# bigomics/plaid

Measured on NVIDIA B200. Metric: plaid() cells x genesets scored/sec, higher is better.
Workload: dtype f64

## Files before the change

### plaid_b200/csrc/api.cu

```cuda
#include <math.h>
#include <stdio.h>
#include <string.h>
#include <stdlib.h>
#include <time.h>
#if defined(__x86_64__)
#include <immintrin.h>
#endif

#include <algorithm>
#include <condition_variable>
#include <functional>
#include <mutex>
#include <new>
#include <thread>

#include "common.cuh"

using namespace plaidgpu;

namespace {

struct DevBuf {
  void* p = nullptr;
  size_t cap = 0;
// ... 667 lines not shown
  CK(c->b_rowb.reserve((size_t)c->P * sizeof(double)));
  const double* dmean = nullptr;
  if (mean_host) {
    CK(cudaMemcpyAsync(c->b_rowb.p, mean_host, (size_t)c->P * sizeof(double), cudaMemcpyHostToDevice, c->stream));
    dmean = c->b_rowb.as<double>();
  }
  CK(launch_row_moments(c->xx, c->P, c->N, dmean, c->b_rowa.as<double>(), c->stream));
  c->launches += 1;
  CK(cudaMemcpyAsync(out_host, c->b_rowa.p, (size_t)c->P * sizeof(double), cudaMemcpyDeviceToHost, c->stream));
  CK(cudaStreamSynchronize(c->stream));
  return PLAIDGPU_OK;
}

bool is_rank_scorer(int s) {
  return s == PLAIDGPU_SING || s == PLAIDGPU_SSGSEA || s == PLAIDGPU_UCELL || s == PLAIDGPU_AUCELL;
}

bool needs_norm(const plaidgpu_opts& o) {
  return (o.scorer == PLAIDGPU_PLAID && o.normalize) || o.scorer == PLAIDGPU_SSGSEA || o.scorer == PLAIDGPU_UCELL ||
         o.scorer == PLAIDGPU_AUCELL || o.scorer == PLAIDGPU_GSVA;
}

double host_value_of(unsigned long long k) {
  const unsigned long long b = (k & 0x8000000000000000ull) ? (k & 0x7fffffffffffffffull) : ~k;
  double d;
  memcpy(&d, &b, sizeof(d));
  return d;
}

int run_colstats(plaidgpu_ctx* c, int which) {
  CK(c->b_med_all.reserve(std::max<int64_t>(c->N, 1) * sizeof(double)));
  CK(c->b_med_nz.reserve(std::max<int64_t>(c->N, 1) * sizeof(double)));
  CK(c->b_colmin.reserve(std::max<int64_t>(c->N, 1) * sizeof(double)));
  CK(c->b_fail.reserve(sizeof(int)));
  CK(c->b_list.reserve(std::max<int64_t>(c->N, 1) * sizeof(int64_t)));
  CK(launch_colstats(c->raw, c->S, c->S, c->N, c->b_med_all.as<double>(), c->b_med_nz.as<double>(),
                     c->b_colmin.as<double>(), c->b_fail.as<int>(), c->b_list.as<int64_t>(), which, c->stream));
  c->launches += 1;
  if (which != COLSTATS_NZ) c->have_all = true;
  if (which != COLSTATS_ALL) c->have_nz = true;
  return PLAIDGPU_OK;
}

void ship_join(plaidgpu_ctx* c) {
  if (!c->shipper.joinable()) return;
  {
    std::lock_guard<std::mutex> lk(c->ship_m);
    c->ship_done = true;
  }
  c->ship_cv.notify_all();
  c->shipper.join();
}
void ship_body(plaidgpu_ctx* c) {
  cudaSetDevice(c->device);
  size_t next = 0;
  for (;;) {
    std::pair<int64_t, int64_t> job;
    {
      std::unique_lock<std::mutex> lk(c->ship_m);
      c->ship_cv.wait(lk, [&] { return next < c->ship_q.size() || c->ship_done; });
      if (next >= c->ship_q.size()) return;
      job = c->ship_q[next];
    }
    cudaStreamWaitEvent(c->copy_stream, c->ev_ship[next], 0);
    cudaMemcpyAsync(c->early_out + job.first * (int64_t)c->S, c->raw + job.first * (int64_t)c->S,
                    (size_t)job.second * c->S * sizeof(double), cudaMemcpyDeviceToHost, c->copy_stream);
    cudaEventRecord(c->ev_early, c->copy_stream);
// ... 1755 lines not shown
  const double* dx = x;
  if (location == PLAIDGPU_HOST) {
    const size_t total = (size_t)S * (size_t)N;
    CK(c->b_raw.reserve(total * sizeof(double)));
    CK(cudaMemcpyAsync(c->b_raw.p, x, total * sizeof(double), cudaMemcpyHostToDevice, c->stream));
    dx = c->b_raw.as<double>();
  }
  return topk_device(c, dx, S, N, k, decreasing != 0, idx, val);
} catch (const std::bad_alloc&) {
  return PLAIDGPU_ERR_NOMEM;
} catch (...) {
  return PLAIDGPU_ERR_ARG;
}

int plaidgpu_normalize_medians(plaidgpu_ctx* c, const double* x, int32_t S, int64_t N, int ignore_zero,
                               int location, double* out) try {
  if (!c) return PLAIDGPU_ERR_ARG;
  if (S <= 0 || N < 0 || (N > 0 && (!x || !out))) return fail(c, PLAIDGPU_ERR_ARG, "bad argument");
  trace("begin");
  CK(cudaSetDevice(c->device));
  c->in_call = false;
  c->computed = false;
  const int64_t total = (int64_t)S * N;
  const double* dx = x;
  if (location == PLAIDGPU_HOST) {
    CK(c->b_raw.reserve((size_t)std::max<int64_t>(total, 1) * sizeof(double)));
    if (total) CK(cudaMemcpyAsync(c->b_raw.p, x, (size_t)total * sizeof(double), cudaMemcpyHostToDevice, c->stream));
    dx = c->b_raw.as<double>();
  }
  CK(c->b_med_all.reserve(std::max<int64_t>(N, 1) * sizeof(double)));
  CK(c->b_med_nz.reserve(std::max<int64_t>(N, 1) * sizeof(double)));
  CK(c->b_colmin.reserve(std::max<int64_t>(N, 1) * sizeof(double)));
  CK(cudaEventRecord(c->ev[2], c->stream));
  CK(c->b_fail.reserve(sizeof(int)));
  CK(c->b_list.reserve(std::max<int64_t>(N, 1) * sizeof(int64_t)));
  const int which = ignore_zero < 0 ? COLSTATS_BOTH : (ignore_zero ? COLSTATS_NZ : COLSTATS_ALL);
  CK(launch_colstats(dx, S, S, N, c->b_med_all.as<double>(), c->b_med_nz.as<double>(), c->b_colmin.as<double>(),
                     c->b_fail.as<int>(), c->b_list.as<int64_t>(), which, c->stream));
  c->launches += 1;
  CK(cudaEventRecord(c->ev[3], c->stream));
  c->h_med_all.resize((size_t)N);
  c->h_med_nz.resize((size_t)N);
  c->h_colmin.resize((size_t)N);
  if (N) {
    CK(cudaMemcpyAsync(c->h_med_all.data(), c->b_med_all.p, (size_t)N * sizeof(double), cudaMemcpyDeviceToHost, c->stream));
    CK(cudaMemcpyAsync(c->h_med_nz.data(), c->b_med_nz.p, (size_t)N * sizeof(double), cudaMemcpyDeviceToHost, c->stream));
    CK(cudaMemcpyAsync(c->h_colmin.data(), c->b_colmin.p, (size_t)N * sizeof(double), cudaMemcpyDeviceToHost, c->stream));
  }
  CK(cudaStreamSynchronize(c->stream));
  float ms = 0.f;
  cudaEventElapsedTime(&ms, c->ev[2], c->ev[3]);
  c->ms[1] = ms;
  double mn = INFINITY;
  for (int64_t j = 0; j < N; ++j) mn = fmin(mn, c->h_colmin[j]);
  plaidgpu_scalars s{};
  plaidgpu_combine_medians(ignore_zero, mn, c->h_med_all.data(), c->h_med_nz.data(), N, &s);
  const double* med = s.ignore_zero ? c->b_med_nz.as<double>() : c->b_med_all.as<double>();
  CK(cudaEventRecord(c->ev[4], c->stream));
  if (location == PLAIDGPU_DEVICE) {
    CK(launch_fixup(dx, out, S, S, 0, N, med, s.med_mean, 1.0, nullptr, c->stream));
    c->launches += 1;
    CK(cudaEventRecord(c->ev[5], c->stream));
  } else {
    CK(launch_fixup(dx, c->b_raw.as<double>(), S, S, 0, N, med, s.med_mean, 1.0, nullptr, c->stream));
    c->launches += 1;
    CK(cudaEventRecord(c->ev[5], c->stream));
    if (total) CK(cudaMemcpyAsync(out, c->b_raw.p, (size_t)total * sizeof(double), cudaMemcpyDeviceToHost, c->stream));
// ... 13 lines not shown
```

### plaid_b200/csrc/stats_kernels.cu

```cuda
#include "common.cuh"

#include <math.h>
#include <stdio.h>
#include <stdlib.h>

namespace plaidgpu {

namespace {

constexpr int NT = 256;
constexpr int NBIN = 2048;
constexpr int NTGT = 4;
constexpr int CAND = 256;
constexpr int NDIG = 6;
constexpr unsigned long long ZERO_KEY = 0x8000000000000000ull;

__device__ __forceinline__ int digit_shift(int d) { return d < 5 ? 53 - 11 * d : 0; }
__device__ __forceinline__ int digit_bits(int d) { return d < 5 ? 11 : 9; }


struct BinHit { int bin; unsigned before, count; };
__device__ BinHit find_bin(const unsigned* __restrict__ hist, int nb, unsigned k, unsigned* __restrict__ part,
                           BinHit* __restrict__ slot) {
  const int tid = threadIdx.x, lane = tid & 31;
  const int per = nb / NT;
  unsigned sum = 0;
  for (int i = 0; i < per; ++i) sum += hist[tid * per + i];
  part[tid] = sum;
  __syncthreads();
  if (tid < 32) {
    unsigned loc = 0;
#pragma unroll
    for (int i = 0; i < NT / 32; ++i) loc += part[lane * (NT / 32) + i];
    unsigned incl = loc;
#pragma unroll
    for (int o = 1; o < 32; o <<= 1) {
      const unsigned v = __shfl_up_sync(FULL, incl, o);
// ... 18 lines not shown

struct StatsSmem {
  unsigned hist[NTGT][NBIN];
  unsigned long long cand[NTGT][CAND];
  unsigned long long prefix[NTGT];
  unsigned long long result[NTGT];
  unsigned k[NTGT];
  unsigned cnt[NTGT];
  unsigned ncand[NTGT];
  int active[NTGT];
  int depth[NTGT];
  unsigned red_u[NT / 32][3];
  unsigned long long red_k[NT / 32];
  unsigned nnan, nzero, nneg;
  unsigned long long minkey;
  unsigned part[NT];
  BinHit hit;
};

__device__ void pick_bin(StatsSmem& s, int g, int d) {
  const BinHit h = find_bin(s.hist[g], 1 << digit_bits(d), s.k[g], s.part, &s.hit);
  __syncthreads();
  if (threadIdx.x == 0) {
    s.prefix[g] |= (unsigned long long)h.bin << digit_shift(d);
    s.k[g] -= h.before;
    s.cnt[g] = h.count;
    s.depth[g] = d + 1;
  }
  __syncthreads();
}

__global__ void __launch_bounds__(NT) k_colstats(const double* __restrict__ x, int64_t ld, int32_t S,
                                                 int64_t N, const int64_t* __restrict__ cols,
                                                 double* __restrict__ med_all,
                                                 double* __restrict__ med_nz,
                                                 double* __restrict__ colmin) {
  extern __shared__ unsigned char smem_raw[];
  StatsSmem& s = *reinterpret_cast<StatsSmem*>(smem_raw);
  const int tid = threadIdx.x, lane = tid & 31, wid = tid >> 5;

  for (int64_t it = blockIdx.x; it < N; it += gridDim.x) {
    const int64_t j = cols ? cols[it] : it;
    const double* __restrict__ c = x + j * ld;

    for (int i = tid; i < NBIN; i += NT) s.hist[0][i] = 0;
    __syncthreads();
    unsigned nnan = 0, nzero = 0;
    unsigned long long mink = ~0ull;
    int runbin = -1;
    unsigned runcnt = 0;
    for (int l = tid; l < S; l += NT) {
      const double v = c[l];
      if (v != v) {
        ++nnan;
        continue;
      }
      const unsigned long long key = key_of(v);
      nzero += (key == ZERO_KEY);
      mink = key < mink ? key : mink;
      const int bin = (int)(key >> 53);
      if (bin != runbin) {
        if (runcnt) atomicAdd(&s.hist[0][runbin], runcnt);
        runbin = bin;
        runcnt = 0;
      }
      ++runcnt;
    }
    if (runcnt) atomicAdd(&s.hist[0][runbin], runcnt);
    __syncthreads();
    unsigned nneg = 0;
    for (int i = tid; i < NBIN / 2; i += NT) nneg += s.hist[0][i];
#pragma unroll
// ... 767 lines not shown
        }
#pragma unroll
        for (int o = 16; o > 0; o >>= 1) {
          le += __shfl_xor_sync(FULL, le, o);
          const unsigned long long t = __shfl_xor_sync(FULL, nx, o);
          nx = t < nx ? t : nx;
        }
        if (lane == 0) {
          atomicAdd(&s.cle, le);
          atomicMin(&s.nxt, nx);
        }
        __syncthreads();
        B = (qb < s.cle) ? A : s.nxt;
      }
    }
    if (tid == 0) {
      if (!good) {
        const int slot = atomicAdd(fail_count, 1);
        fail_list[slot] = j;
      } else {
        double m = NZ ? 0.0 : nan("");
        if (count > 0) {
          const double a = value_of(A), b = value_of(B);
          m = (count & 1u) ? a : (a + b) / 2.0;
        }
        med[j] = m;
        colmin[j] = s.minkey != ~0ull ? value_of(s.minkey) : INFINITY;
      }
    }
    __syncthreads();
  }
}

__global__ void __launch_bounds__(256) k_fixup(const double* __restrict__ x, double* __restrict__ out,
                                               int64_t ld, int32_t S, int64_t j0, int64_t j1,
                                               const double* __restrict__ med, double c, double alpha,
                                               const double* __restrict__ beta) {
  for (int64_t j = j0 + blockIdx.x; j < j1; j += gridDim.x) {
    const double shift = (med ? -med[j] : 0.0) + c;
    const double* __restrict__ xi = x + j * ld;
    double* __restrict__ oi = out + j * ld;
    const bool vec = ((((uintptr_t)xi) | ((uintptr_t)oi)) & 15) == 0;
    if (vec) {
      const int S2 = S >> 1;
      const double2* __restrict__ x2 = reinterpret_cast<const double2*>(xi);
      double2* __restrict__ o2 = reinterpret_cast<double2*>(oi);
      for (int l = threadIdx.x; l < S2; l += blockDim.x) {
        double2 v = __ldcs(x2 + l);
        v.x = __dmul_rn(alpha, __dadd_rn(v.x, shift));
        v.y = __dmul_rn(alpha, __dadd_rn(v.y, shift));
        if (beta) {
          v.x = __dadd_rn(v.x, beta[2 * l]);
          v.y = __dadd_rn(v.y, beta[2 * l + 1]);
        }
        __stcs(o2 + l, v);
      }
      if ((S & 1) && threadIdx.x == 0) {
        double v = __dmul_rn(alpha, __dadd_rn(xi[S - 1], shift));
        if (beta) v = __dadd_rn(v, beta[S - 1]);
        oi[S - 1] = v;
      }
    } else {
      for (int l = threadIdx.x; l < S; l += blockDim.x) {
        double v = __dmul_rn(alpha, __dadd_rn(xi[l], shift));
        if (beta) v = __dadd_rn(v, beta[l]);
        oi[l] = v;
// ... 106 lines not shown
  out[0] = res[0] == ~0ull ? INFINITY : value_of(res[0]);
  out[1] = res[1] == 0ull ? -INFINITY : value_of(res[1]);
}

}

bool colstats_small(int32_t S) { return S < 4 * SAMP; }

cudaError_t launch_colstats(const double* x, int64_t ld, int32_t S, int64_t N, double* med_all,
                            double* med_nz, double* colmin, int* d_fail, int64_t* d_list, int which, cudaStream_t st) {
  if (N <= 0) return cudaSuccess;
  {
    cudaError_t e = cudaFuncSetAttribute(k_colstats, cudaFuncAttributeMaxDynamicSharedMemorySize,
                                         (int)sizeof(StatsSmem));
    if (e != cudaSuccess) return e;
    const void* fast[3] = {(const void*)k_colstats_fast<true, true>, (const void*)k_colstats_fast<true, false>,
                           (const void*)k_colstats_fast<false, true>};
    for (int i = 0; i < 3; ++i) {
      e = cudaFuncSetAttribute(fast[i], cudaFuncAttributeMaxDynamicSharedMemorySize,
                               (int)(i == 0 ? sizeof(Stats2Smem) : STATS2_SMEM_ONE));
      if (e != cudaSuccess) return e;
    }
    e = cudaFuncSetAttribute(k_colstats_one<false>, cudaFuncAttributeMaxDynamicSharedMemorySize, (int)sizeof(Stats3Smem));
    if (e != cudaSuccess) return e;
    e = cudaFuncSetAttribute(k_colstats_one<true>, cudaFuncAttributeMaxDynamicSharedMemorySize, (int)sizeof(Stats3Smem));
    if (e != cudaSuccess) return e;
  }
  int dev = 0, sms = 148;
  cudaGetDevice(&dev);
  cudaDeviceGetAttribute(&sms, cudaDevAttrMultiProcessorCount, dev);
  if (S < 4 * SAMP) {
    int64_t grid = (int64_t)sms * 4;
    if (grid > N) grid = N;
    k_colstats<<<(unsigned)grid, NT, sizeof(StatsSmem), st>>>(x, ld, S, N, nullptr, med_all, med_nz, colmin);
    return cudaGetLastError();
  }
  cudaError_t e = launch_fill_u32(d_fail, 0u, 1, st);
  if (e != cudaSuccess) return e;
  int per_sm = 1;
  static const bool old_one = getenv("PLAIDGPU_COLSTATS_OLD") != nullptr;
  if (which != COLSTATS_BOTH && !old_one) {
    const size_t sm3 = sizeof(Stats3Smem);
    if (which == COLSTATS_ALL) cudaOccupancyMaxActiveBlocksPerMultiprocessor(&per_sm, k_colstats_one<false>, NT, sm3);
    else cudaOccupancyMaxActiveBlocksPerMultiprocessor(&per_sm, k_colstats_one<true>, NT, sm3);
    if (per_sm < 1) per_sm = 1;
    int64_t grid = (int64_t)sms * per_sm;
    if (grid > N) grid = N;
    if (which == COLSTATS_ALL)
      k_colstats_one<false><<<(unsigned)grid, NT, sm3, st>>>(x, ld, S, N, med_all, colmin, d_fail, d_list);
    else
      k_colstats_one<true><<<(unsigned)grid, NT, sm3, st>>>(x, ld, S, N, med_nz, colmin, d_fail, d_list);
    e = cudaGetLastError();
    if (e != cudaSuccess) return e;
  } else {
  const size_t smem = which == COLSTATS_BOTH ? sizeof(Stats2Smem) : STATS2_SMEM_ONE;
  if (which == COLSTATS_ALL)
    cudaOccupancyMaxActiveBlocksPerMultiprocessor(&per_sm, k_colstats_fast<true, false>, NT, smem);
  else if (which == COLSTATS_NZ)
    cudaOccupancyMaxActiveBlocksPerMultiprocessor(&per_sm, k_colstats_fast<false, true>, NT, smem);
  else
    cudaOccupancyMaxActiveBlocksPerMultiprocessor(&per_sm, k_colstats_fast<true, true>, NT, smem);
  if (per_sm < 1) per_sm = 1;
  int64_t grid = (int64_t)sms * per_sm;
  if (grid > N) grid = N;
  if (which == COLSTATS_ALL)
    k_colstats_fast<true, false><<<(unsigned)grid, NT, smem, st>>>(x, ld, S, N, med_all, med_nz, colmin, d_fail, d_list);
  else if (which == COLSTATS_NZ)
    k_colstats_fast<false, true><<<(unsigned)grid, NT, smem, st>>>(x, ld, S, N, med_all, med_nz, colmin, d_fail, d_list);
  else
    k_colstats_fast<true, true><<<(unsigned)grid, NT, smem, st>>>(x, ld, S, N, med_all, med_nz, colmin, d_fail, d_list);
  e = cudaGetLastError();
  if (e != cudaSuccess) return e;
  }
  int nfail = 0;
  e = cudaMemcpyAsync(&nfail, d_fail, sizeof(int), cudaMemcpyDeviceToHost, st);
  if (e != cudaSuccess) return e;
  e = cudaStreamSynchronize(st);
  if (e != cudaSuccess) return e;
  if (getenv("PLAIDGPU_TRACE_COLSTATS"))
    fprintf(stderr, "[plaidgpu] colstats: %d of %lld columns redone by the three-pass kernel\n", nfail, (long long)N);
  if (nfail > 0) {
    int64_t g2 = (int64_t)sms * 4;
    if (g2 > nfail) g2 = nfail;
    k_colstats<<<(unsigned)g2, NT, sizeof(StatsSmem), st>>>(x, ld, S, nfail, d_list, med_all, med_nz, colmin);
    e = cudaGetLastError();
    if (e != cudaSuccess) return e;
  }
  return cudaSuccess;
}

cudaError_t launch_fixup(const double* x, double* out, int64_t ld, int32_t S, int64_t j0, int64_t j1,
                         const double* med, double c, double alpha, const double* beta,
                         cudaStream_t st) {
  if (j1 <= j0) return cudaSuccess;
  int dev = 0, sms = 148;
  cudaGetDevice(&dev);
  cudaDeviceGetAttribute(&sms, cudaDevAttrMultiProcessorCount, dev);
  if (ld == S && (S & 1) == 0 && S >= FIX_CHUNK && ((((uintptr_t)(x + j0 * ld)) | ((uintptr_t)(out + j0 * ld))) & 15) == 0) {
    const int64_t chunks = ((j1 - j0) * (int64_t)S + FIX_CHUNK - 1) / FIX_CHUNK;
    int64_t grid = (int64_t)sms * 8;
    if (grid > chunks) grid = chunks;
    k_fixup_flat<<<(unsigned)grid, 256, 0, st>>>(x, out, S, j0, j1, med, c, alpha, beta);
    return cudaGetLastError();
  }
  int64_t grid = (int64_t)sms * 8;
  if (grid > j1 - j0) grid = j1 - j0;
  k_fixup<<<(unsigned)grid, 256, 0, st>>>(x, out, ld, S, j0, j1, med, c, alpha, beta);
  return cudaGetLastError();
}

cudaError_t launch_group_stats(const double* x, int64_t ld, int32_t S, int K, const int32_t* cols, const int32_t* seg,
                               int nchunk, double* partial, double* out, cudaStream_t st, bool fix, const double* med,
                               double c, double alpha, const double* beta) {
  if (S <= 0 || K <= 0) return cudaSuccess;
  dim3 g((unsigned)((int64_t)nchunk * K), (unsigned)((S + 255) / 256));
  if (fix) k_group_partial<true><<<g, 256, 0, st>>>(x, ld, S, cols, seg, partial, med, c, alpha, beta);
  else k_group_partial<false><<<g, 256, 0, st>>>(x, ld, S, cols, seg, partial, nullptr, 0.0, 1.0, nullptr);
  cudaError_t e = cudaGetLastError();
  if (e != cudaSuccess) return e;
  const int64_t width = (int64_t)K * 2 * S;
  k_group_combine<<<(unsigned)((width + 255) / 256), 256, 0, st>>>(partial, width, nchunk, out);
// ... 25 lines not shown
```

### plaid_b200/csrc/tail_kernels.cu

```cuda
#include "common.cuh"

namespace plaidgpu {

namespace {

constexpr int TAIL_WARPS = 32;

__global__ void __launch_bounds__(1024) k_tile_scan(uint32_t* __restrict__ cnt, int32_t Pt, uint32_t* __restrict__ rowptr,
                                                    uint32_t* __restrict__ total) {
  __shared__ uint32_t wsum[32];
  const int t = blockIdx.x, tid = threadIdx.x, lane = tid & 31, w = tid >> 5;
  uint32_t* __restrict__ c = cnt + (size_t)t * Pt;
  uint32_t* __restrict__ rp = rowptr + (size_t)t * (Pt + 1);
  const int per = (Pt + 1023) / 1024;
  const int lo = min(Pt, tid * per), hi = min(Pt, lo + per);
  uint32_t s = 0;
  for (int i = lo; i < hi; ++i) s += c[i];
  uint32_t incl = s;
#pragma unroll
  for (int o = 1; o < 32; o <<= 1) {
    const uint32_t v = __shfl_up_sync(FULL, incl, o);
    if (lane >= o) incl += v;
  }
  if (lane == 31) wsum[w] = incl;
// ... 48 lines not shown
    for (int32_t e0 = xp[j]; e0 < e1; e0 += 128) {
      int32_t rr[4], gg[4];
      double xv[4];
      uint32_t pos[4];
#pragma unroll
      for (int u = 0; u < 4; ++u) {
        const int32_t e = e0 + 32 * u + lane;
        const bool in = e < e1;
        rr[u] = in ? __ldg(oi + e) : -1;
        xv[u] = in ? __ldg(ox + e) : 0.0;
      }
#pragma unroll
      for (int u = 0; u < 4; ++u) gg[u] = rr[u] >= 0 ? __ldg(tmap + rr[u]) : -1;
#pragma unroll
      for (int u = 0; u < 4; ++u)
        if (gg[u] >= 0) pos[u] = base + rp[gg[u]] + atomicAdd(cur + gg[u], 1u);
#pragma unroll
      for (int u = 0; u < 4; ++u) {
        if (gg[u] < 0) continue;
        double v = xform_value(mode, xv[u], a0, a1);
        if (mode >= XF_SING) v -= fb;
        const int32_t q = (int32_t)__double2ll_rn(v * sc);
        if (q == 0 && v != 0.0 && skip_if) atomicExch(const_cast<int*>(skip_if), 1);
        ent[pos[u]] = make_uint2((uint32_t)q, cell);
      }
    }
  }
}

__global__ void __launch_bounds__(256) k_fill_u32(uint32_t* __restrict__ p, uint32_t v, int64_t n) {
  for (int64_t i = blockIdx.x * (int64_t)blockDim.x + threadIdx.x; i < n; i += (int64_t)gridDim.x * blockDim.x) p[i] = v;
}

struct TailParams {
  const uint32_t* tptr;
  const uint16_t* tidx;
  const int32_t* sorder;
  const uint32_t* rowptr;
  const uint32_t* total;
  const uint2* ent;
  int32_t S, Pt, C, tiles;
  long long* tmp;
  int64_t ld;
  unsigned int* counter;
  const int* skip_if;
};

__global__ void __launch_bounds__(TAIL_WARPS * 32, 1) k_tail(const TailParams p) {
  if (p.skip_if && *p.skip_if != 0) return;
  extern __shared__ uint32_t tail_sm[];
  const int lane = threadIdx.x & 31, w = threadIdx.x >> 5;
  const int C = p.C;
  uint32_t* __restrict__ lo = tail_sm + (size_t)w * C;
  short* __restrict__ hi = reinterpret_cast<short*>(tail_sm + (size_t)TAIL_WARPS * C) + (size_t)w * C;
  for (int c = lane; c < C; c += 32) {
    lo[c] = 0u;
    hi[c] = 0;
  }
  __syncwarp();
  const uint32_t lo_sa = (uint32_t)__cvta_generic_to_shared(lo), hi_sa = (uint32_t)__cvta_generic_to_shared(hi);
  const unsigned nitems = (unsigned)p.tiles * (unsigned)p.S;
  for (;;) {
    unsigned item = 0;
    if (lane == 0) item = atomicAdd(p.counter, 1u);
    item = __shfl_sync(FULL, item, 0);
    if (item >= nitems) break;
    const int t = (int)(item / (unsigned)p.S);
    const int s = p.sorder[item - (unsigned)t * (unsigned)p.S];
    const uint32_t* __restrict__ rp = p.rowptr + (size_t)t * (p.Pt + 1);
    uint32_t base = 0;
    for (int u = lane; u < t; u += 32) base += p.total[u];
#pragma unroll
    for (int o = 16; o > 0; o >>= 1) base += __shfl_xor_sync(FULL, base, o);
    const uint2* __restrict__ ent = p.ent + base;
    const uint32_t m0 = p.tptr[s], m1 = p.tptr[s + 1];
    for (uint32_t mb = m0; mb < m1; mb += 32) {
      uint32_t r0 = 0, rn = 0;
      if (mb + lane < m1) {
        const uint32_t g = p.tidx[mb + lane];
        r0 = rp[g];
        rn = rp[g + 1] - r0;
      }
      const int cnt = (int)min(32u, m1 - mb);
      auto add = [&](const uint2 rec) {
        if (rec.y != 0xFFFFu) {
          const uint32_t a = lo_sa + rec.y * 4u;
          uint32_t old;
          asm volatile("ld.shared.u32 %0, [%1];" : "=r"(old) : "r"(a) : "memory");
          const uint32_t nv = old + rec.x;
          asm volatile("st.shared.u32 [%0], %1;" ::"r"(a), "r"(nv) : "memory");
          if ((nv < rec.x) != ((int32_t)rec.x < 0)) {
            const uint32_t ah = hi_sa + rec.y * 2u;
            short hv;
            asm volatile("ld.shared.s16 %0, [%1];" : "=h"(hv) : "r"(ah) : "memory");
            hv = (short)(hv + ((nv < rec.x) ? 1 : -1));
            asm volatile("st.shared.s16 [%0], %1;" ::"r"(ah), "h"(hv) : "memory");
          }
        }
        __syncwarp();
      };
      auto prefetch = [&](int kk, uint2& rec, uint32_t& nk, uint32_t& pk) {
        nk = kk < cnt ? __shfl_sync(FULL, rn, kk & 31) : 0u;
        pk = __shfl_sync(FULL, r0, kk & 31);
        rec = make_uint2(0u, 0xFFFFu);
        if ((uint32_t)lane < nk) rec = __ldg(ent + pk + lane);
      };
      auto seg = [&](uint32_t off, uint32_t nk, uint32_t pk) {
        uint2 r = make_uint2(0u, 0xFFFFu);
        if (off + lane < nk) r = __ldg(ent + pk + off + lane);
        return r;
      };
      auto member = [&](const uint2 rec, uint32_t nk, uint32_t pk) {
        if (nk <= 32u) {
          add(rec);
          return;
        }
        uint2 q1 = seg(32u, nk, pk), q2 = seg(64u, nk, pk), q3 = seg(96u, nk, pk);
        add(rec);
        for (uint32_t off = 32; off < nk; off += 96) {
          const uint2 a = q1, b = q2, c = q3;
          q1 = seg(off + 96u, nk, pk);
          q2 = seg(off + 128u, nk, pk);
          q3 = seg(off + 160u, nk, pk);
          add(a);
          if (off + 32u < nk) add(b);
          if (off + 64u < nk) add(c);
        }
      };
      uint2 e0, e1, e2, e3;
      uint32_t n0, n1, n2, n3, p0, p1, p2, p3;
      prefetch(0, e0, n0, p0);
      prefetch(1, e1, n1, p1);
      prefetch(2, e2, n2, p2);
      prefetch(3, e3, n3, p3);
      for (int k = 0; k < cnt; k += 4) {
        member(e0, n0, p0);
        prefetch(k + 4, e0, n0, p0);
        member(e1, n1, p1);
        prefetch(k + 5, e1, n1, p1);
        member(e2, n2, p2);
        prefetch(k + 6, e2, n2, p2);
        member(e3, n3, p3);
        prefetch(k + 7, e3, n3, p3);
      }
    }
    long long* __restrict__ o = p.tmp + (size_t)s * p.ld + (size_t)t * C;
    for (int c = lane; c < C; c += 32) {
      const long long v = ((long long)hi[c] << 32) | (long long)lo[c];
      lo[c] = 0u;
      hi[c] = 0;
      __stcs(o + c, v);
    }
    __syncwarp();
  }
}

}

cudaError_t launch_fill_u32(void* p, uint32_t v, int64_t n, cudaStream_t st) {
  if (n <= 0) return cudaSuccess;
  int64_t grid = (n + 255) / 256;
  if (grid > 148 * 8) grid = 148 * 8;
  k_fill_u32<<<(unsigned)grid, 256, 0, st>>>(static_cast<uint32_t*>(p), v, n);
  return cudaGetLastError();
}

int tail_tile_cells() { return 1056; }

size_t tail_smem_bytes() { return (size_t)TAIL_WARPS * tail_tile_cells() * 6; }

cudaError_t launch_tile_scan(uint32_t* cnt, int32_t Pt, int tiles, uint32_t* rowptr, uint32_t* total, cudaStream_t st) {
  if (tiles <= 0) return cudaSuccess;
  k_tile_scan<<<(unsigned)tiles, 1024, 0, st>>>(cnt, Pt, rowptr, total);
  return cudaGetLastError();
}

cudaError_t launch_tile_place(const int32_t* xp, const int32_t* xe, const int32_t* oi, const double* ox, const double* r0,
                              const int32_t* tmap, const double* colinv, int64_t N, int mode, double a0, double a1,
                              int32_t Pt, const uint32_t* rowptr, const uint32_t* total, uint32_t* cnt, uint2* ent,
                              const int* skip_if, cudaStream_t st) {
  if (N <= 0) return cudaSuccess;
  int64_t grid = (N + 7) / 8;
  if (grid > 148 * 16) grid = 148 * 16;
  k_tile_place<<<(unsigned)grid, 256, 0, st>>>(xp, xe, oi, ox, r0, tmap, colinv, N, mode, a0, a1, Pt, tail_tile_cells(),
                                               rowptr, total, cnt, ent, skip_if);
  return cudaGetLastError();
}

cudaError_t launch_tail(const uint32_t* tptr, const uint16_t* tidx, const int32_t* sorder, const uint32_t* rowptr,
                        const uint32_t* total, const uint2* ent, int32_t S, int32_t Pt, int tiles,
                        long long* tmp, unsigned int* counter, const int* skip_if, cudaStream_t st) {
  if (tiles <= 0 || S <= 0) return cudaSuccess;
  TailParams p{};
  p.tptr = tptr;
  p.tidx = tidx;
  p.sorder = sorder;
  p.rowptr = rowptr;
  p.total = total;
  p.ent = ent;
  p.S = S;
  p.Pt = Pt;
  p.C = tail_tile_cells();
// ... 19 lines not shown
```

Baseline: 46.33 billion.

## Add warp-per-column median kernel and launch fallback without host sync

Adds a one-warp-per-column median/min kernel. It estimates a float bracket from a 1024-element sample, streams each column once while collecting candidates into shared memory, and resolves the median with warp-level radix narrowing. Columns are handed out dynamically through an atomic counter, and the next column's sample is prefetched. The fallback three-pass kernel now reads the failure count from device memory instead of copying it to the host and synchronizing, so it is always launched, sometimes with no work. This removes a host round-trip and improves load balance, at the cost of more complex code and possible candidate overflow fallbacks.

```diff
diff --git a/plaid_b200/csrc/api.cu b/plaid_b200/csrc/api.cu
--- a/plaid_b200/csrc/api.cu
+++ b/plaid_b200/csrc/api.cu
@@ -723,7 +723,7 @@
   CK(c->b_med_all.reserve(std::max<int64_t>(c->N, 1) * sizeof(double)));
   CK(c->b_med_nz.reserve(std::max<int64_t>(c->N, 1) * sizeof(double)));
   CK(c->b_colmin.reserve(std::max<int64_t>(c->N, 1) * sizeof(double)));
-  CK(c->b_fail.reserve(sizeof(int)));
+  CK(c->b_fail.reserve(4 * sizeof(int)));
   CK(c->b_list.reserve(std::max<int64_t>(c->N, 1) * sizeof(int64_t)));
   CK(launch_colstats(c->raw, c->S, c->S, c->N, c->b_med_all.as<double>(), c->b_med_nz.as<double>(),
                      c->b_colmin.as<double>(), c->b_fail.as<int>(), c->b_list.as<int64_t>(), which, c->stream));
@@ -2545,7 +2545,7 @@
   CK(c->b_med_nz.reserve(std::max<int64_t>(N, 1) * sizeof(double)));
   CK(c->b_colmin.reserve(std::max<int64_t>(N, 1) * sizeof(double)));
   CK(cudaEventRecord(c->ev[2], c->stream));
-  CK(c->b_fail.reserve(sizeof(int)));
+  CK(c->b_fail.reserve(4 * sizeof(int)));
   CK(c->b_list.reserve(std::max<int64_t>(N, 1) * sizeof(int64_t)));
   const int which = ignore_zero < 0 ? COLSTATS_BOTH : (ignore_zero ? COLSTATS_NZ : COLSTATS_ALL);
   CK(launch_colstats(dx, S, S, N, c->b_med_all.as<double>(), c->b_med_nz.as<double>(), c->b_colmin.as<double>(),
diff --git a/plaid_b200/csrc/stats_kernels.cu b/plaid_b200/csrc/stats_kernels.cu
--- a/plaid_b200/csrc/stats_kernels.cu
+++ b/plaid_b200/csrc/stats_kernels.cu
@@ -1,8 +1,10 @@
 #include "common.cuh"
 
+#include <float.h>
 #include <math.h>
 #include <stdio.h>
 #include <stdlib.h>
+#include <string.h>
 
 namespace plaidgpu {
 
@@ -87,12 +89,14 @@
 
 __global__ void __launch_bounds__(NT) k_colstats(const double* __restrict__ x, int64_t ld, int32_t S,
                                                  int64_t N, const int64_t* __restrict__ cols,
+                                                 const int* __restrict__ ncols,
                                                  double* __restrict__ med_all,
                                                  double* __restrict__ med_nz,
                                                  double* __restrict__ colmin) {
   extern __shared__ unsigned char smem_raw[];
   StatsSmem& s = *reinterpret_cast<StatsSmem*>(smem_raw);
   const int tid = threadIdx.x, lane = tid & 31, wid = tid >> 5;
+  if (ncols) N = *ncols;
 
   for (int64_t it = blockIdx.x; it < N; it += gridDim.x) {
     const int64_t j = cols ? cols[it] : it;
@@ -926,6 +930,305 @@
   }
 }
 
+constexpr int WCAND = 3072;
+constexpr int WB = 16;
+constexpr int WARP_MAX_S = 32768;
+constexpr int WARPS_PER_SM = 11;
+
+struct alignas(16) WarpSmem {
+  unsigned hist[256];
+  unsigned small[32];
+  unsigned key[WCAND + 1];
+  unsigned short row[WCAND + 1];
+};
+
+__device__ __forceinline__ unsigned fkey_canon(float f) { return fkey_of(f == 0.f ? 0.f : f); }
+
+template <class Each>
+__device__ __forceinline__ void warp_narrow(unsigned* hist, Each each, int hi, unsigned& pref, unsigned& pmask,
+                                            unsigned& k, unsigned& n) {
+  const int lane = threadIdx.x & 31;
+  uint4* const h4 = reinterpret_cast<uint4*>(hist);
+  while (n > 32 && hi >= 0) {
+    const int nb = hi + 1 < 8 ? hi + 1 : 8, sh = hi + 1 - nb;
+    const unsigned dm = (1u << nb) - 1u;
+    h4[lane] = make_uint4(0u, 0u, 0u, 0u);
+    h4[lane + 32] = make_uint4(0u, 0u, 0u, 0u);
+    __syncwarp();
+    each([&](unsigned key) {
+      if ((key & pmask) == pref) atomicAdd(&hist[(key >> sh) & dm], 1u);
+    });
+    __syncwarp();
+    const uint4 a = h4[2 * lane], b = h4[2 * lane + 1];
+    const unsigned cnt[8] = {a.x, a.y, a.z, a.w, b.x, b.y, b.z, b.w};
+    unsigned sum = 0;
+#pragma unroll
+    for (int i = 0; i < 8; ++i) sum += cnt[i];
+    unsigned incl = sum;
+#pragma unroll
+    for (int o = 1; o < 32; o <<= 1) {
+      const unsigned v = __shfl_up_sync(FULL, incl, o);
+      if (lane >= o) incl += v;
+    }
+    const int l = __ffs(__ballot_sync(FULL, k < incl)) - 1;
+    unsigned before = incl - sum, bin = 8 * lane + 7, c = cnt[7];
+    bool found = false;
+#pragma unroll
+    for (int i = 0; i < 8; ++i) {
+      if (found) continue;
+      if (k < before + cnt[i]) {
+        found = true;
+        bin = 8 * lane + i;
+        c = cnt[i];
+      } else {
+        before += cnt[i];
+      }
+    }
+    bin = __shfl_sync(FULL, bin, l);
+    before = __shfl_sync(FULL, before, l);
+    c = __shfl_sync(FULL, c, l);
+    pref |= bin << sh;
+    pmask |= dm << sh;
+    k -= before;
+    n = c;
+    hi = sh - 1;
+    __syncwarp();
+  }
+}
+
+template <class K>
+__device__ __forceinline__ unsigned warp_rank_lanes(K mine, unsigned n, unsigned k) {
+  const unsigned lane = threadIdx.x & 31;
+  unsigned r = 0;
+  for (unsigned u = 0; u < n; ++u) {
+    const K o = __shfl_sync(FULL, mine, u);
+    r += (o < mine) || (o == mine && u < lane);
+  }
+  return __ballot_sync(FULL, lane < n && r == k);
+}
+
+__device__ __forceinline__ unsigned long long warp_min_u64(unsigned long long v) {
+#pragma unroll
+  for (int o = 16; o > 0; o >>= 1) {
+    const unsigned long long t = __shfl_xor_sync(FULL, v, o);
+    v = t < v ? t : v;
+  }
+  return v;
+}
+
+template <bool NZ>
+__global__ void __launch_bounds__(32, WARPS_PER_SM) k_colstats_warp(const double* __restrict__ x, int64_t ld, int32_t S, int64_t N,
+                                                      double* __restrict__ med, double* __restrict__ colmin,
+                                                      int* __restrict__ fail_count, int64_t* __restrict__ fail_list,
+                                                      unsigned long long* __restrict__ next_col) {
+  __shared__ WarpSmem s;
+  const int lane = threadIdx.x;
+  const unsigned ltm = (1u << lane) - 1u;
+
+  double sv[32];
+  auto load_sample = [&](int64_t jj) {
+    const double* __restrict__ c = x + jj * ld;
+#pragma unroll
+    for (int t = 0; t < 32; ++t) sv[t] = c[(int)(((int64_t)(lane + 32 * t) * S) / SAMP)];
+  };
+  int64_t j = blockIdx.x;
+  if (j < N) load_sample(j);
+  while (j < N) {
+    const double* __restrict__ c = x + j * ld;
+
+    unsigned sk[32], mv = 0, kmin = ~0u, kmax = 0u;
+#pragma unroll
+    for (int t = 0; t < 32; ++t) {
+      const double v = sv[t];
+      const bool valid = (v == v) && !(NZ && v == 0.0);
+      const unsigned k = valid ? fkey_canon(__double2float_rn(v)) : ~0u;
+      sk[t] = k;
+      mv += valid;
+      if (valid) {
+        kmin = min(kmin, k);
+        kmax = max(kmax, k);
+      }
+    }
+    const unsigned mcount = __reduce_add_sync(FULL, mv);
+    kmin = __reduce_min_sync(FULL, kmin);
+    kmax = __reduce_max_sync(FULL, kmax);
+    float lof = -FLT_MAX, hif = FLT_MAX;
+    if (mcount >= 48) {
+      const double mid = 0.5 * (double)(mcount - 1);
+      const double delta = 1.25 * sqrt((double)mcount) + 2.0;
+      const int a = (int)floor(mid - delta), b = (int)ceil(mid + delta);
+      const int top = 31 - __clz((int)((kmin ^ kmax) | 1u));
+      auto sample_key = [&](unsigned r) -> unsigned {
+        unsigned pref = 0, pmask = 0, k = r, n = mcount;
+        warp_narrow(
+            s.hist,
+            [&](auto&& f) {
+#pragma unroll
+              for (int t = 0; t < 32; ++t)
+                if (sk[t] != ~0u) f(sk[t]);
+            },
+            top, pref, pmask, k, n);
+        if (n > 32) return (kmin & ~pmask) | pref;
+        unsigned base = 0;
+#pragma unroll
+        for (int t = 0; t < 32; ++t) {
+          const bool m = sk[t] != ~0u && (sk[t] & pmask) == pref;
+          const unsigned bal = __ballot_sync(FULL, m);
+          if (m) s.small[base + __popc(bal & ltm)] = sk[t];
+          base += __popc(bal);
+        }
+        __syncwarp();
+        const unsigned mine = lane < (int)n ? s.small[lane] : ~0u;
+        const unsigned res = __shfl_sync(FULL, mine, __ffs(warp_rank_lanes(mine, n, k)) - 1);
+        __syncwarp();
+        return res;
+      };
+#pragma unroll 1
+      for (int e = 0; e < 2; ++e) {
+        if (e == 0 ? a < 0 : b > (int)mcount - 1) continue;
+        const unsigned key = sample_key((unsigned)(e == 0 ? a : b));
+        const float f = fvalue_of(e == 0 ? key & ~1023u : key | 1023u);
+        if (f == f) {
+          if (e == 0) lof = fmaxf(f, -FLT_MAX);
+          else hif = fminf(f, FLT_MAX);
+        }
+      }
+    }
+
+    const bool zin = NZ && lof <= 0.f && hif >= 0.f;
+    unsigned bel = 0, nz = 0, nc = 0;
+    double minv = INFINITY;
+    auto visit = [&](double v, int row) {
+      const float f = __double2float_rn(v);
+      minv = v < minv ? v : minv;
+      const bool lt = f < lof;
+      bool cd = !(lt || f > hif);
+      if (NZ) {
+        const unsigned hi = (unsigned)__double2hiint(v), lo = (unsigned)__double2loint(v);
+        const bool isz = ((hi + hi) | lo) == 0u;
+        nz += isz;
+        cd = cd && !(zin && isz);
+      }
+      bel += lt;
+      const unsigned m = __ballot_sync(FULL, cd);
+      const unsigned p = nc + __popc(m & ltm);
+      const unsigned q = cd && p < (unsigned)WCAND ? p : (unsigned)WCAND;
+      s.key[q] = __float_as_uint(f);
+      s.row[q] = (unsigned short)row;
+      nc += __popc(m);
+    };
+    const int h = (int)((reinterpret_cast<uintptr_t>(c) >> 3) & 1);
+    const int np = (S - h) >> 1;
+    const double2* __restrict__ c2 = reinterpret_cast<const double2*>(c + h);
+    if (h) visit(lane == 0 ? c[0] : INFINITY, 0);
+    constexpr int RING = 32 * WB;
+    const double2 pad = make_double2(INFINITY, INFINITY);
+    double2 v[WB];
+#pragma unroll
+    for (int u = 0; u < WB; ++u) v[u] = 32 * u + lane < np ? __ldcs(c2 + 32 * u + lane) : pad;
+    for (int base = 0; base < np; base += RING) {
+#pragma unroll
+      for (int u = 0; u < WB; ++u) {
+        const int r = h + 2 * (base + 32 * u + lane);
+        visit(v[u].x, r);
+        visit(v[u].y, r + 1);
+        const int pn = base + RING + 32 * u + lane;
+        v[u] = pn < np ? __ldcs(c2 + pn) : pad;
+      }
+    }
+    if ((S - h) & 1) visit(lane == 0 ? c[S - 1] : INFINITY, S - 1);
+
+    unsigned long long jn = 0;
+    if (lane == 0) jn = gridDim.x + atomicAdd(next_col, 1ull);
+    jn = __shfl_sync(FULL, jn, 0);
+    if ((int64_t)jn < N) load_sample((int64_t)jn);
+
+    bel = __reduce_add_sync(FULL, bel);
+    if (NZ) {
+      nz = __reduce_add_sync(FULL, nz);
+      if (lof > 0.f) bel -= nz;
+    }
+    const unsigned long long mink = warp_min_u64(minv == INFINITY ? ~0ull : key_of(minv));
+    const unsigned count = (unsigned)S - (NZ ? nz : 0u);
+    const unsigned ka = count ? (count - 1) / 2 : 0, kb = count / 2;
+    bool good = nc <= (unsigned)WCAND && (count == 0 || (ka >= bel && kb < bel + nc));
+    unsigned long long A = 0, B = 0;
+    if (good && count > 0) {
+      bool nan_seen = false;
+      for (unsigned i = lane; i < nc; i += 32) {
+        const float f = __uint_as_float(s.key[i]);
+        nan_seen |= f != f;
+        s.key[i] = fkey_canon(f);
+      }
+      __syncwarp();
+      good = !__any_sync(FULL, nan_seen);
+      const unsigned klo = fkey_canon(lof), khi = fkey_canon(hif);
+      const int top = 31 - __clz((int)((klo ^ khi) | 1u));
+      auto select = [&](unsigned q, bool next, unsigned long long& ra, unsigned long long& rb, bool& have_b) -> bool {
+        unsigned pref = 0, pmask = 0, k = q, n = nc;
+        warp_narrow(
+            s.hist,
+            [&](auto&& f) {
+              for (unsigned i = lane; i < nc; i += 32) f(s.key[i]);
+            },
+            top, pref, pmask, k, n);
+        if (n <= 32) {
+          unsigned base = 0;
+          for (unsigned i0 = 0; i0 < nc && base < n; i0 += 32) {
+            const unsigned i = i0 + lane;
+            const bool m = i < nc && (s.key[i] & pmask) == pref;
+            const unsigned bal = __ballot_sync(FULL, m);
+            if (m) s.small[base + __popc(bal & ltm)] = s.row[i];
+            base += __popc(bal);
+          }
+          __syncwarp();
+          const unsigned long long mine = lane < (int)n ? key_of(c[s.small[lane]]) : ~0ull;
+          ra = __shfl_sync(FULL, mine, __ffs(warp_rank_lanes(mine, n, k)) - 1);
+          have_b = next && k + 1 < n;
+          if (have_b) rb = __shfl_sync(FULL, mine, __ffs(warp_rank_lanes(mine, n, k + 1)) - 1);
+          __syncwarp();
+          return true;
+        }
+        unsigned long long mn = ~0ull, mx = 0;
+        for (unsigned i = lane; i < nc; i += 32)
+          if ((s.key[i] & pmask) == pref) {
+            const unsigned long long kk = key_of(c[s.row[i]]);
+            mn = kk < mn ? kk : mn;
+            mx = kk > mx ? kk : mx;
+          }
+        mn = warp_min_u64(mn);
+        mx = ~warp_min_u64(~mx);
+        ra = rb = mn;
+        have_b = next && k + 1 < n;
+        return mn == mx;
+      };
+      if (good) {
+        const unsigned qa = ka - bel, qb = kb - bel;
+        bool have_b = false;
+        good = select(qa, qb != qa, A, B, have_b);
+        if (qb == qa) B = A;
+        else if (good && !have_b) good = select(qb, false, B, B, have_b);
+      }
+    }
+    if (lane == 0) {
+      if (!good) {
+        const int slot = atomicAdd(fail_count, 1);
+        fail_list[slot] = j;
+      } else {
+        double m = NZ ? 0.0 : nan("");
+        if (count > 0) {
+          const double a = value_of(A), b = value_of(B);
+          m = (count & 1u) ? a : (a + b) / 2.0;
+        }
+        med[j] = m;
+        colmin[j] = mink != ~0ull ? value_of(mink) : INFINITY;
+      }
+    }
+    __syncwarp();
+    j = (int64_t)jn;
+  }
+}
+
 __global__ void __launch_bounds__(256) k_fixup(const double* __restrict__ x, double* __restrict__ out,
                                                int64_t ld, int32_t S, int64_t j0, int64_t j1,
                                                const double* __restrict__ med, double c, double alpha,
@@ -1098,14 +1401,30 @@
   if (S < 4 * SAMP) {
     int64_t grid = (int64_t)sms * 4;
     if (grid > N) grid = N;
-    k_colstats<<<(unsigned)grid, NT, sizeof(StatsSmem), st>>>(x, ld, S, N, nullptr, med_all, med_nz, colmin);
+    k_colstats<<<(unsigned)grid, NT, sizeof(StatsSmem), st>>>(x, ld, S, N, nullptr, nullptr, med_all, med_nz, colmin);
     return cudaGetLastError();
   }
-  cudaError_t e = launch_fill_u32(d_fail, 0u, 1, st);
+  cudaError_t e = launch_fill_u32(d_fail, 0u, 4, st);
   if (e != cudaSuccess) return e;
   int per_sm = 1;
-  static const bool old_one = getenv("PLAIDGPU_COLSTATS_OLD") != nullptr;
-  if (which != COLSTATS_BOTH && !old_one) {
+  const char* ab = getenv("PLAIDGPU_COLSTATS_OLD");
+  const int old = !ab ? 0 : (strcmp(ab, "one") == 0 ? 1 : 2);
+  if (which != COLSTATS_BOTH && old == 0 && S <= WARP_MAX_S) {
+    const void* kw = which == COLSTATS_ALL ? (const void*)k_colstats_warp<false> : (const void*)k_colstats_warp<true>;
+    e = cudaFuncSetAttribute(kw, cudaFuncAttributePreferredSharedMemoryCarveout, cudaSharedmemCarveoutMaxShared);
+    if (e != cudaSuccess) return e;
+    cudaOccupancyMaxActiveBlocksPerMultiprocessor(&per_sm, kw, 32, 0);
+    if (per_sm < 1) per_sm = 1;
+    int64_t grid = (int64_t)sms * per_sm;
+    if (grid > N) grid = N;
+    unsigned long long* next = reinterpret_cast<unsigned long long*>(d_fail + 2);
+    if (which == COLSTATS_ALL)
+      k_colstats_warp<false><<<(unsigned)grid, 32, 0, st>>>(x, ld, S, N, med_all, colmin, d_fail, d_list, next);
+    else
+      k_colstats_warp<true><<<(unsigned)grid, 32, 0, st>>>(x, ld, S, N, med_nz, colmin, d_fail, d_list, next);
+    e = cudaGetLastError();
+    if (e != cudaSuccess) return e;
+  } else if (which != COLSTATS_BOTH && old != 2) {
     const size_t sm3 = sizeof(Stats3Smem);
     if (which == COLSTATS_ALL) cudaOccupancyMaxActiveBlocksPerMultiprocessor(&per_sm, k_colstats_one<false>, NT, sm3);
     else cudaOccupancyMaxActiveBlocksPerMultiprocessor(&per_sm, k_colstats_one<true>, NT, sm3);
@@ -1119,40 +1438,37 @@
     e = cudaGetLastError();
     if (e != cudaSuccess) return e;
   } else {
-  const size_t smem = which == COLSTATS_BOTH ? sizeof(Stats2Smem) : STATS2_SMEM_ONE;
-  if (which == COLSTATS_ALL)
-    cudaOccupancyMaxActiveBlocksPerMultiprocessor(&per_sm, k_colstats_fast<true, false>, NT, smem);
-  else if (which == COLSTATS_NZ)
-    cudaOccupancyMaxActiveBlocksPerMultiprocessor(&per_sm, k_colstats_fast<false, true>, NT, smem);
-  else
-    cudaOccupancyMaxActiveBlocksPerMultiprocessor(&per_sm, k_colstats_fast<true, true>, NT, smem);
-  if (per_sm < 1) per_sm = 1;
-  int64_t grid = (int64_t)sms * per_sm;
-  if (grid > N) grid = N;
-  if (which == COLSTATS_ALL)
-    k_colstats_fast<true, false><<<(unsigned)grid, NT, smem, st>>>(x, ld, S, N, med_all, med_nz, colmin, d_fail, d_list);
-  else if (which == COLSTATS_NZ)
-    k_colstats_fast<false, true><<<(unsigned)grid, NT, smem, st>>>(x, ld, S, N, med_all, med_nz, colmin, d_fail, d_list);
-  else
-    k_colstats_fast<true, true><<<(unsigned)grid, NT, smem, st>>>(x, ld, S, N, med_all, med_nz, colmin, d_fail, d_list);
-  e = cudaGetLastError();
-  if (e != cudaSuccess) return e;
-  }
-  int nfail = 0;
-  e = cudaMemcpyAsync(&nfail, d_fail, sizeof(int), cudaMemcpyDeviceToHost, st);
-  if (e != cudaSuccess) return e;
-  e = cudaStreamSynchronize(st);
-  if (e != cudaSuccess) return e;
-  if (getenv("PLAIDGPU_TRACE_COLSTATS"))
-    fprintf(stderr, "[plaidgpu] colstats: %d of %lld columns redone by the three-pass kernel\n", nfail, (long long)N);
-  if (nfail > 0) {
-    int64_t g2 = (int64_t)sms * 4;
-    if (g2 > nfail) g2 = nfail;
-    k_colstats<<<(unsigned)g2, NT, sizeof(StatsSmem), st>>>(x, ld, S, nfail, d_list, med_all, med_nz, colmin);
+    const size_t smem = which == COLSTATS_BOTH ? sizeof(Stats2Smem) : STATS2_SMEM_ONE;
+    if (which == COLSTATS_ALL)
+      cudaOccupancyMaxActiveBlocksPerMultiprocessor(&per_sm, k_colstats_fast<true, false>, NT, smem);
+    else if (which == COLSTATS_NZ)
+      cudaOccupancyMaxActiveBlocksPerMultiprocessor(&per_sm, k_colstats_fast<false, true>, NT, smem);
+    else
+      cudaOccupancyMaxActiveBlocksPerMultiprocessor(&per_sm, k_colstats_fast<true, true>, NT, smem);
+    if (per_sm < 1) per_sm = 1;
+    int64_t grid = (int64_t)sms * per_sm;
+    if (grid > N) grid = N;
+    if (which == COLSTATS_ALL)
+      k_colstats_fast<true, false><<<(unsigned)grid, NT, smem, st>>>(x, ld, S, N, med_all, med_nz, colmin, d_fail, d_list);
+    else if (which == COLSTATS_NZ)
+      k_colstats_fast<false, true><<<(unsigned)grid, NT, smem, st>>>(x, ld, S, N, med_all, med_nz, colmin, d_fail, d_list);
+    else
+      k_colstats_fast<true, true><<<(unsigned)grid, NT, smem, st>>>(x, ld, S, N, med_all, med_nz, colmin, d_fail, d_list);
     e = cudaGetLastError();
     if (e != cudaSuccess) return e;
   }
-  return cudaSuccess;
+  if (getenv("PLAIDGPU_TRACE_COLSTATS")) {
+    int nfail = 0;
+    e = cudaMemcpyAsync(&nfail, d_fail, sizeof(int), cudaMemcpyDeviceToHost, st);
+    if (e == cudaSuccess) e = cudaStreamSynchronize(st);
+    if (e != cudaSuccess) return e;
+    fprintf(stderr, "[plaidgpu] colstats: %d of %lld columns redone by the three-pass kernel (first pass: %d CTAs per SM)\n",
+            nfail, (long long)N, per_sm);
+  }
+  int64_t g2 = (int64_t)sms * 4;
+  if (g2 > N) g2 = N;
+  k_colstats<<<(unsigned)g2, NT, sizeof(StatsSmem), st>>>(x, ld, S, N, d_list, d_fail, med_all, med_nz, colmin);
+  return cudaGetLastError();
 }
 
 cudaError_t launch_fixup(const double* x, double* out, int64_t ld, int32_t S, int64_t j0, int64_t j1,
```

Result: slower. 44.97 billion (median of 6 runs) (-2.9%).

## Flatten member segments into warp-wide stream with shared atomics for tail accumulation

Applied to the files above, without the earlier changes.

The tail kernel's per-member segment walk is replaced by a warp prefix scan over member segment lengths, so all entries of a 32-member block stream contiguously in 32-lane chunks. Lanes map to segments through a shuffle and ballot lookup. Accumulation now uses shared atomic adds with carry propagation into packed biased 16-bit high words, where before it used a load/store pair under a syncwarp. The flush vectorizes into 128-bit stores. This targets lane underutilization on short segments and per-add syncwarp serialization, at the cost of extra shuffles per chunk, per-warp scratch shared memory, and atomic contention.

```diff
diff --git a/plaid_b200/csrc/tail_kernels.cu b/plaid_b200/csrc/tail_kernels.cu
--- a/plaid_b200/csrc/tail_kernels.cu
+++ b/plaid_b200/csrc/tail_kernels.cu
@@ -104,6 +104,18 @@
   for (int64_t i = blockIdx.x * (int64_t)blockDim.x + threadIdx.x; i < n; i += (int64_t)gridDim.x * blockDim.x) p[i] = v;
 }
 
+constexpr uint32_t HI_BIAS = 0x8000u, HI_BIAS2 = 0x80008000u;
+
+__device__ __forceinline__ void acc_add(uint32_t lo_sa, uint32_t hi_sa, const uint2 rec) {
+  const uint32_t q = rec.x, c = rec.y;
+  uint32_t old, d;
+  asm volatile("atom.shared.add.u32 %0, [%1], %2;" : "=r"(old) : "r"(lo_sa + c * 4u), "r"(q) : "memory");
+  asm("{\n\t.reg .u32 t;\n\tadd.cc.u32 t, %1, %2;\n\taddc.u32 %0, %3, 0;\n\t}"
+      : "=r"(d) : "r"(old), "r"(q), "r"((uint32_t)((int32_t)q >> 31)));
+  asm volatile("{\n\t.reg .pred p;\n\tsetp.ne.u32 p, %1, 0;\n\t@p red.shared.add.u32 [%0], %2;\n\t}"
+               ::"r"(hi_sa + (c & ~1u) * 2u), "r"(d), "r"(__funnelshift_l(0u, d, c << 4)) : "memory");
+}
+
 struct TailParams {
   const uint32_t* tptr;
   const uint16_t* tidx;
@@ -124,13 +136,18 @@
   const int lane = threadIdx.x & 31, w = threadIdx.x >> 5;
   const int C = p.C;
   uint32_t* __restrict__ lo = tail_sm + (size_t)w * C;
-  short* __restrict__ hi = reinterpret_cast<short*>(tail_sm + (size_t)TAIL_WARPS * C) + (size_t)w * C;
-  for (int c = lane; c < C; c += 32) {
-    lo[c] = 0u;
-    hi[c] = 0;
+  uint32_t* __restrict__ hiw = tail_sm + (size_t)TAIL_WARPS * C + (size_t)w * (C / 2);
+  uint2* __restrict__ scr = reinterpret_cast<uint2*>(tail_sm + (size_t)TAIL_WARPS * C * 3 / 2) + w * 32;
+  for (int c = lane; c < C / 2; c += 32) {
+    lo[2 * c] = 0u;
+    lo[2 * c + 1] = 0u;
+    hiw[c] = HI_BIAS2;
   }
   __syncwarp();
-  const uint32_t lo_sa = (uint32_t)__cvta_generic_to_shared(lo), hi_sa = (uint32_t)__cvta_generic_to_shared(hi);
+  const uint32_t lo_sa = (uint32_t)__cvta_generic_to_shared(lo), hi_sa = (uint32_t)__cvta_generic_to_shared(hiw);
+  uint32_t le, lt;
+  asm("mov.u32 %0, %%lanemask_le;" : "=r"(le));
+  asm("mov.u32 %0, %%lanemask_lt;" : "=r"(lt));
   const unsigned nitems = (unsigned)p.tiles * (unsigned)p.S;
   for (;;) {
     unsigned item = 0;
@@ -144,7 +161,8 @@
     for (int u = lane; u < t; u += 32) base += p.total[u];
 #pragma unroll
     for (int o = 16; o > 0; o >>= 1) base += __shfl_xor_sync(FULL, base, o);
-    const uint2* __restrict__ ent = p.ent + base;
+    const uint2* ent = p.ent + base + lane;
+    asm("mov.b64 %0, %0;" : "+l"(ent));
     const uint32_t m0 = p.tptr[s], m1 = p.tptr[s + 1];
     for (uint32_t mb = m0; mb < m1; mb += 32) {
       uint32_t r0 = 0, rn = 0;
@@ -153,75 +171,54 @@
         r0 = rp[g];
         rn = rp[g + 1] - r0;
       }
-      const int cnt = (int)min(32u, m1 - mb);
-      auto add = [&](const uint2 rec) {
-        if (rec.y != 0xFFFFu) {
-          const uint32_t a = lo_sa + rec.y * 4u;
-          uint32_t old;
-          asm volatile("ld.shared.u32 %0, [%1];" : "=r"(old) : "r"(a) : "memory");
-          const uint32_t nv = old + rec.x;
-          asm volatile("st.shared.u32 [%0], %1;" ::"r"(a), "r"(nv) : "memory");
-          if ((nv < rec.x) != ((int32_t)rec.x < 0)) {
-            const uint32_t ah = hi_sa + rec.y * 2u;
-            short hv;
-            asm volatile("ld.shared.s16 %0, [%1];" : "=h"(hv) : "r"(ah) : "memory");
-            hv = (short)(hv + ((nv < rec.x) ? 1 : -1));
-            asm volatile("st.shared.s16 [%0], %1;" ::"r"(ah), "h"(hv) : "memory");
-          }
-        }
-        __syncwarp();
+      uint32_t incl = rn;
+#pragma unroll
+      for (int o = 1; o < 32; o <<= 1) {
+        const uint32_t v = __shfl_up_sync(FULL, incl, o);
+        if (lane >= o) incl += v;
+      }
+      const uint32_t total = __shfl_sync(FULL, incl, 31);
+      if (total == 0u) continue;
+      const uint32_t ne = __ballot_sync(FULL, rn != 0u);
+      __syncwarp();
+      if (rn != 0u) scr[__popc(ne & lt)] = make_uint2(incl - rn, r0 - (incl - rn));
+      __syncwarp();
+      const uint2 so = scr[lane];
+      const uint32_t start = (uint32_t)lane < (uint32_t)__popc(ne) ? so.x : 0xFFFFFFFFu, off = so.y;
+      int before = -1;
+      auto fetch = [&](uint32_t P0) {
+        uint32_t bit;
+        asm("shl.b32 %0, 1, %1;" : "=r"(bit) : "r"(start - P0));
+        const uint32_t m = __reduce_or_sync(FULL, bit);
+        const uint32_t o = __shfl_sync(FULL, off, before + __popc(m & le));
+        before += __popc(m);
+        uint2 rec = make_uint2(0u, (uint32_t)lane);
+        if (P0 + lane < total) rec = __ldg(ent + (o + P0));
+        return rec;
       };
-      auto prefetch = [&](int kk, uint2& rec, uint32_t& nk, uint32_t& pk) {
-        nk = kk < cnt ? __shfl_sync(FULL, rn, kk & 31) : 0u;
-        pk = __shfl_sync(FULL, r0, kk & 31);
-        rec = make_uint2(0u, 0xFFFFu);
-        if ((uint32_t)lane < nk) rec = __ldg(ent + pk + lane);
-      };
-      auto seg = [&](uint32_t off, uint32_t nk, uint32_t pk) {
-        uint2 r = make_uint2(0u, 0xFFFFu);
-        if (off + lane < nk) r = __ldg(ent + pk + off + lane);
-        return r;
-      };
-      auto member = [&](const uint2 rec, uint32_t nk, uint32_t pk) {
-        if (nk <= 32u) {
-          add(rec);
-          return;
-        }
-        uint2 q1 = seg(32u, nk, pk), q2 = seg(64u, nk, pk), q3 = seg(96u, nk, pk);
-        add(rec);
-        for (uint32_t off = 32; off < nk; off += 96) {
-          const uint2 a = q1, b = q2, c = q3;
-          q1 = seg(off + 96u, nk, pk);
-          q2 = seg(off + 128u, nk, pk);
-          q3 = seg(off + 160u, nk, pk);
-          add(a);
-          if (off + 32u < nk) add(b);
-          if (off + 64u < nk) add(c);
-        }
-      };
-      uint2 e0, e1, e2, e3;
-      uint32_t n0, n1, n2, n3, p0, p1, p2, p3;
-      prefetch(0, e0, n0, p0);
-      prefetch(1, e1, n1, p1);
-      prefetch(2, e2, n2, p2);
-      prefetch(3, e3, n3, p3);
-      for (int k = 0; k < cnt; k += 4) {
-        member(e0, n0, p0);
-        prefetch(k + 4, e0, n0, p0);
-        member(e1, n1, p1);
-        prefetch(k + 5, e1, n1, p1);
-        member(e2, n2, p2);
-        prefetch(k + 6, e2, n2, p2);
-        member(e3, n3, p3);
-        prefetch(k + 7, e3, n3, p3);
-      }
-    }
+      uint2 q0 = fetch(0u), q1 = fetch(32u), q2 = fetch(64u);
+      for (uint32_t P0 = 0;; P0 += 96u) {
+        acc_add(lo_sa, hi_sa, q0);
+        q0 = fetch(P0 + 96u);
+        if (P0 + 32u >= total) break;
+        acc_add(lo_sa, hi_sa, q1);
+        q1 = fetch(P0 + 128u);
+        if (P0 + 64u >= total) break;
+        acc_add(lo_sa, hi_sa, q2);
+        q2 = fetch(P0 + 160u);
+        if (P0 + 96u >= total) break;
+      }
+    }
+    __syncwarp();
     long long* __restrict__ o = p.tmp + (size_t)s * p.ld + (size_t)t * C;
-    for (int c = lane; c < C; c += 32) {
-      const long long v = ((long long)hi[c] << 32) | (long long)lo[c];
-      lo[c] = 0u;
-      hi[c] = 0;
-      __stcs(o + c, v);
+    for (int c = lane; c < C / 2; c += 32) {
+      const uint2 l = *reinterpret_cast<const uint2*>(lo + 2 * c);
+      const uint32_t h = hiw[c];
+      const long long v0 = (long long)(((uint64_t)(h & 0xFFFFu) - HI_BIAS) << 32) + l.x;
+      const long long v1 = (long long)(((uint64_t)(h >> 16) - HI_BIAS) << 32) + l.y;
+      *reinterpret_cast<uint2*>(lo + 2 * c) = make_uint2(0u, 0u);
+      hiw[c] = HI_BIAS2;
+      __stcs(reinterpret_cast<longlong2*>(o + 2 * c), make_longlong2(v0, v1));
     }
     __syncwarp();
   }
@@ -239,7 +236,7 @@
 
 int tail_tile_cells() { return 1056; }
 
-size_t tail_smem_bytes() { return (size_t)TAIL_WARPS * tail_tile_cells() * 6; }
+size_t tail_smem_bytes() { return (size_t)TAIL_WARPS * (tail_tile_cells() * 6 + 32 * sizeof(uint2)); }
 
 cudaError_t launch_tile_scan(uint32_t* cnt, int32_t Pt, int tiles, uint32_t* rowptr, uint32_t* total, cudaStream_t st) {
   if (tiles <= 0) return cudaSuccess;
```

Result: faster. 46.17 billion before, 51.00 billion after (median of 6 runs) (+10.5%).
